# sksundaram-learning/linkerd

Hardware: AMD Instinct MI355X
Metric: histogram samples ingested+summarized/sec (1M series) and % HBM peak (higher is better)
Workload: dtype u32; 1 GPU; C3: 1M series, 1e9 Zipf(s=1) samples per step, log-normal values; series_total=1000000, series_per_gpu=1000000, rotating_batches=3, parallelism=series-sharded x1 (weighted ranges), step=ingest (sample+plan+bin1+bin2) + snapshot(reset, dense counts + summaries)

## Files before the change

### linkerd_amd/csrc/l5dh_ingest.hip

```cpp
#include <algorithm>
#include <type_traits>

#include "l5dh_device.hpp"

namespace l5dh {
namespace {

constexpr uint32_t RSAMPLE = 1u << 18;
#ifndef L5DH_RS_WG
#define L5DH_RS_WG 64
#endif
constexpr int RS_WG = L5DH_RS_WG;
static_assert((RSAMPLE + RS_WG - 1) / RS_WG <= 65535, "k_rsample's u16 LDS counters: at most 65535 draws per workgroup");
constexpr uint32_t INVALID = 0xFFFFFFFFu;

__device__ __forceinline__ uint32_t round_up(uint32_t x, uint32_t m) { return (x + m - 1) / m * m; }

__device__ __forceinline__ uint32_t rcap(double prev, double e, double s, bool exact, double pad, uint32_t align,
                                         uint32_t pct, double z, bool floor_sample) {
  double c;
  if (exact) {
    c = e;
  } else {
    const double e0 = prev / s, sg = sqrt(e0 + 1.0);
    const double r = sqrt(e + 1.0) + 0.5 * z;
    const double sb = !floor_sample && prev == 0.0 && e == 0.0 ? ceil(4.0 * s) : ceil(r * r * s);
    if (prev > 0.0 && e >= e0 - 6.0 * sg && (floor_sample || e <= e0 + 4.0 * sg)) {
      c = ceil(prev * 1.0625 + 4.0 * sqrt(prev));
      if (floor_sample) c = fmax(c, sb);
    } else {
      c = sb;
    }
    c += pad;
  }
  if (pct != 100) c = floor(c * (double)pct / 100.0);
  return round_up((uint32_t)fmin(c, 1073741824.0), align);
}

__device__ __forceinline__ uint64_t block_excl_scan64(uint64_t v, uint64_t* lds , uint64_t* total) {
  const int lane = threadIdx.x & 63, w = threadIdx.x >> 6;
  const uint64_t incl = wave_incl_scan(v);
  if (lane == 63) lds[w] = incl;
  __syncthreads();
  if (threadIdx.x == 0) {
    uint64_t acc = 0;
    for (int k = 0; k < 16; ++k) {
      const uint64_t q = lds[k];
      lds[k] = acc;
      acc += q;
    }
    lds[16] = acc;
  }
  __syncthreads();
  const uint64_t r = lds[w] + incl - v;
  *total = lds[16];
  __syncthreads();
  return r;
}

#ifdef L5DH_PHASES
__device__ unsigned long long g_phase_plan[16];
#define RP_MARK(k) \
  if (threadIdx.x == 0) g_phase_plan[k] = wall_clock64();
#define RS_MARK(k) \
  if (threadIdx.x == 0 && blockIdx.x == 0) g_phase_plan[k] = wall_clock64();
#else
#define RP_MARK(k)
#define RS_MARK(k)
#endif

__global__ __launch_bounds__(1024) void k_rsample(const uint32_t* __restrict__ series, size_t n, uint32_t S, uint32_t K,
                                                  uint32_t* __restrict__ kest) {
  extern __shared__ uint32_t c[];
  RS_MARK(8)
  for (uint32_t i = threadIdx.x; i < (K + 1) / 2; i += 1024) c[i] = 0;
  __syncthreads();
  RS_MARK(9)
  const uint64_t m = n < RSAMPLE ? n : RSAMPLE;
  const uint64_t per = (m + RS_WG - 1) / RS_WG;
  const uint64_t k0 = blockIdx.x * per, k1 = k0 + per < m ? k0 + per : m;
  for (uint64_t kb = k0; kb < k1; kb += 4 * 1024) {
    uint32_t sv[4];
#pragma unroll
    for (int u = 0; u < 4; ++u) {
      const uint64_t k = kb + threadIdx.x + 1024u * u;
      const uint64_t i = m == n ? k : k * n / m;
      sv[u] = k < k1 ? series[i < n ? i : 0] : 0xFFFFFFFFu;
    }
#pragma unroll
    for (int u = 0; u < 4; ++u)
      if (sv[u] < S) {
        const uint32_t key = sv[u] >> 4;
        atomicAdd(&c[key >> 1], (key & 1u) ? 0x10000u : 1u);
      }
  }
  __syncthreads();
  RS_MARK(10)
  for (uint32_t i = threadIdx.x; i < (K + 1) / 2; i += 1024) {
    const uint32_t x = c[i];
    if (x & 0xFFFFu) atomicAdd(&kest[2 * i], x & 0xFFFFu);
    if ((x >> 16) && 2 * i + 1 < K) atomicAdd(&kest[2 * i + 1], x >> 16);
  }
  RS_MARK(11)
}

constexpr size_t RPLAN1_LDS = 32768 * 4;
constexpr uint32_t RFIX2_ONE_WG_MAX = 16384;
__global__ __launch_bounds__(1024) void k_rplan1(size_t n, uint32_t F, const uint32_t* __restrict__ kest,
                                                 const uint32_t* __restrict__ kprev, uint32_t* __restrict__ meta,
                                                 size_t cap32, size_t dlim16, uint32_t thr_min, uint32_t dmax,
                                                 uint32_t pct) {
  __shared__ uint32_t lh[33];
  __shared__ uint32_t sthr;
  __shared__ uint4 lds4[17];
  __shared__ uint64_t l64[17];
  __shared__ uint32_t dl[DIRECT_MAX + 1];
  __shared__ uint32_t capl[BIN1_BINS];
  extern __shared__ uint32_t tw[];
  const MetaLayout L = meta_layout(F);
  const uint32_t FS = (F + ST_TILES - 1) / ST_TILES;
  const uint32_t NW = (F + 31) / 32;
  const uint64_t m = n < RSAMPLE ? n : RSAMPLE;
  const bool exact = m == n;
  const double s = m ? (double)n / (double)m : 1.0;
  const uint32_t j = threadIdx.x, t0 = j * 32;
  const int lane = lane_id();
  RP_MARK(0)
  if (j < 33) lh[j] = 0;
  capl[j] = 0;
  auto load_pairs = [&](const uint32_t* __restrict__ kw, uint4 (&x)[16]) {
#pragma unroll
    for (int i = 0; i < 16; ++i) {
      const uint32_t t = 2u * (j + 1024u * (uint32_t)i);
      x[i] = make_uint4(0u, 0u, 0u, 0u);
      if (t + 1 < F) {
        x[i] = *reinterpret_cast<const uint4*>(kw + 2 * t);
      } else if (t < F) {
        x[i].x = kw[2 * t];
        x[i].y = kw[2 * t + 1];
      }
    }
  };
  uint2 te[16];
  {
    uint4 x[16];
    load_pairs(kest, x);
#pragma unroll
    for (int i = 0; i < 16; ++i) te[i] = make_uint2(x[i].x + x[i].y, x[i].z + x[i].w);
  }
  auto scaled = [&](uint32_t v) -> uint32_t { return (uint32_t)fmin((double)v * s, 4294967295.0); };
  __syncthreads();
  RP_MARK(1)
  auto hist = [&](uint32_t v) {
    const uint32_t e = scaled(v);
    const bool ok = dmax > 0 && e >= thr_min && e > 0;
    const int bin = ok ? 31 - __clz((int)e) : 0;
    const uint64_t act = __ballot(ok);
    if (!act) return;
    const int b0 = __builtin_amdgcn_readlane(bin, __builtin_ctzll(act));
    if (__ballot(ok && bin == b0) == act) {
      if (lane == 0) atomicAdd(&lh[b0], (uint32_t)__popcll(act));
    } else if (ok) {
      atomicAdd(&lh[bin], 1u);
    }
  };
#pragma unroll
  for (int i = 0; i < 16; ++i) {
    hist(te[i].x);
    hist(te[i].y);
  }
  __syncthreads();
  if (j < 64) {
    const uint32_t c = j < 32 ? lh[31 - j] : 0u;
    const uint32_t cum = wave_incl_scan32(c);
    const uint64_t ok = __ballot(dmax > 0 && j < 32 && cum <= dmax);
    const int nb = __popcll(ok);
    if (j == 0) sthr = nb ? max(max(thr_min, 1u), 1u << (32 - nb)) : 0xFFFFFFFFu;
  }
#pragma unroll
  for (int i = 0; i < 16; ++i) reinterpret_cast<uint2*>(tw)[j + 1024u * (uint32_t)i] = te[i];
  uint4 xp[16];
  load_pairs(kprev, xp);
  __syncthreads();
  const uint32_t thr = sthr;
  RP_MARK(2)
  uint32_t dbits = 0, E = 0;
#pragma unroll
  for (int k = 0; k < 32; ++k) {
    const uint32_t kk = (uint32_t)(k + (int)j) & 31u;
    const uint32_t v = tw[t0 + kk];
    if (t0 + kk < F && scaled(v) >= thr) dbits |= 1u << kk;
    else E += v;
  }
  __syncthreads();
#pragma unroll
  for (int i = 0; i < 16; ++i)
    reinterpret_cast<uint2*>(tw)[j + 1024u * (uint32_t)i] = make_uint2(xp[i].x + xp[i].y, xp[i].z + xp[i].w);
  __syncthreads();
  uint64_t P = 0;
#pragma unroll
  for (int k = 0; k < 32; ++k) {
    const uint32_t kk = (uint32_t)(k + (int)j) & 31u;
    if (!((dbits >> kk) & 1u)) P += tw[t0 + kk];
  }
  RP_MARK(3)
  uint32_t cv[4] = {(uint32_t)__popc(dbits), 0u, 0u, 0u}, ct[4];
  block_excl_scan4<1024>(cv, lds4, ct);
  const uint32_t ND = ct[0];
  meta[L.dbits() + j] = j < NW ? dbits : 0u;
  meta[L.dpre() + j] = cv[0];
  {
    uint32_t x = dbits, di = cv[0];
    while (x) {
      const uint32_t k = (uint32_t)(__ffs((int)x) - 1);
      x &= x - 1u;
      dl[di] = t0 + k;
      meta[L.dlist() + di] = t0 + k;
      ++di;
    }
  }
  P += __shfl_xor(P, 1, 64);
  E += __shfl_xor(E, 1, 64);
  RP_MARK(4)
  if ((j & 1u) == 0 && (j >> 1) < FS) {
    const uint32_t b = j >> 1;
    capl[b] = rcap((double)P, (double)E, s, exact, 256.0, 4, pct, 6.0, true);
    meta[L.btot() + b] = (uint32_t)min(P, (uint64_t)0xFFFFFFFFu);
  }
  __syncthreads();
  RP_MARK(5)
  const uint32_t TB = FS + 2 * ND;
  if (j >= FS && j < TB) {
    const uint32_t t = dl[(j - FS) >> 1], h = (j - FS) & 1u;
    const double p = (double)kprev[2 * t + h], e = (double)kest[2 * t + h];
    capl[j] = rcap(p, e, s, exact, 256.0, 8, pct, 5.0, false);
  }
  __syncthreads();
  const bool stb = j < FS, dj = j >= FS && j < TB;
  uint64_t tot32, tot16;
  const uint64_t base32 = block_excl_scan64(stb ? (uint64_t)capl[j] : 0ull, l64, &tot32);
  const uint64_t base16 = block_excl_scan64(dj ? (uint64_t)capl[j] : 0ull, l64, &tot16);
  const uint64_t base = stb ? base32 : base16;
  const uint64_t lim = stb ? cap32 : dlim16;
  if (base + capl[j] + 16 > lim)
    capl[j] = base + 16 < lim ? (uint32_t)(lim - 16 - base) & (stb ? ~3u : ~7u) : 0u;
  meta[L.bbase() + j] = (uint32_t)base;
  meta[L.bcap() + j] = j < TB ? capl[j] : 0u;
  meta[L.bcnt() + j] = 0u;
  if (j == 0) {
    uint32_t* hdr = meta + L.hdr();
    hdr[H_ND] = ND;
    hdr[H_OV1] = 0;
    hdr[H_REDO1] = 0;
    hdr[H_OV2] = 0;
    hdr[H_REDO2] = 0;
    hdr[H_COUNT2] = 0;
    hdr[H_EXACT] = exact ? 1u : 0u;
    hdr[H_D16] = (uint32_t)min(tot16, (uint64_t)dlim16);
  }
  RP_MARK(6)
}

#ifdef L5DH_PHASES
__device__ unsigned long long g_phase1[1024 * 8];
__device__ unsigned long long g_phase3[1024 * 8];
#define PH_INIT                                                            \
  const bool ph_on = threadIdx.x == 0 || threadIdx.x == NT1 - 64;          \
  uint32_t ph_acc[8] = {0, 0, 0, 0, 0, 0, 0, 0}, ph_t = (uint32_t)wall_clock64();
#define PH_VWAIT asm volatile("s_waitcnt vmcnt(0)" ::: "memory");
#define PH_MARK(k)                                 \
  if (ph_on) {                                     \
    const uint32_t ph_n = (uint32_t)wall_clock64(); \
    ph_acc[k] += ph_n - ph_t;                      \
    ph_t = ph_n;                                   \
  }
#define PH_FLUSH                                                                          \
  if (ph_on && pass == 0 && (threadIdx.x == 0 || gridDim.x <= 256)) {                      \
    const uint32_t ph_row = blockIdx.x + (threadIdx.x ? 512u : 0u);                       \
    for (int k = 0; k < 7; ++k) g_phase1[ph_row * 8 + k] += ph_acc[k];                    \
    g_phase1[ph_row * 8 + 7] += 1;                                                        \
    if (gridDim.x <= 256) {                                                               \
      g_phase1[(768 + blockIdx.x) * 8 + (threadIdx.x ? 1 : 0)] += ph_acc[7];              \
      if (threadIdx.x == 0) g_phase1[(768 + blockIdx.x) * 8 + 7] += 1;                    \
    }                                                                                     \
  }
#else
#define PH_INIT
#define PH_MARK(k)
#define PH_VWAIT
#define PH_FLUSH
#endif
__device__ __forceinline__ uint4 ld_stream(const uint32_t* p) { return *reinterpret_cast<const uint4*>(p); }
constexpr int CHW = 16384;
constexpr int NT1 = 1024;
constexpr int B1_PT = CHW / NT1;
constexpr int B1_PH = B1_PT / 2;
constexpr int B1_GS = 4;
constexpr int B1_HG = B1_PH / 4;
static_assert(B1_PH % 4 == 0 && B1_PH % B1_GS == 0 && B1_GS % 4 == 0, "halves of whole 16-B groups");
static_assert(NT1 == BIN1_BINS, "one bin per thread");
constexpr uint32_t DSUM_PMAX = 1u << 17;
static_assert(DSUM_PMAX == 1u << 17, "the ranking loop tests the bits of 2^17f, 0x48000000");
constexpr uint32_t NODEST = 0xFFFFFFFFu - (uint32_t)CHW;
constexpr int DSUM_N = DIRECT_MAX * TILE;

struct Bin1Lds {
  static constexpr int DW_N = 1024;
  static constexpr size_t o_stage = 0;
  static constexpr size_t o_cnt = o_stage + CHW * 4;
  static constexpr size_t o_offr = o_cnt + BIN1_BINS * 4;
  static constexpr size_t o_rdelta = o_offr + BIN1_BINS * 4;
  static constexpr size_t o_heads = o_rdelta + BIN1_BINS * 4;
  static constexpr size_t o_gpre = o_heads + CHW / 32 * 4;
  static constexpr size_t o_dw = o_gpre + CHW / 64 * 2;
  static constexpr size_t o_lut2 = o_dw + DW_N * 8;
  static constexpr size_t o_dsum = o_lut2 + LUT2_N * 8;
  static constexpr size_t o_dacc = o_dsum + DSUM_N * 4;
  static constexpr size_t o_breg = o_dacc + BIN1_BINS * 4;
  static constexpr size_t bytes = o_breg + BIN1_BINS * 8;

  template <typename T>
  static __device__ __forceinline__ T* at(uint32_t* smem, size_t o) {
    return reinterpret_cast<T*>(reinterpret_cast<char*>(smem) + o);
  }
  static __device__ __forceinline__ uint32_t* stage(uint32_t* smem) { return at<uint32_t>(smem, o_stage); }
  static __device__ __forceinline__ uint32_t* cnt(uint32_t* smem) { return at<uint32_t>(smem, o_cnt); }
  static __device__ __forceinline__ uint32_t* offr(uint32_t* smem) { return at<uint32_t>(smem, o_offr); }
  static __device__ __forceinline__ uint32_t* rdelta(uint32_t* smem) { return at<uint32_t>(smem, o_rdelta); }
  static __device__ __forceinline__ uint32_t* heads(uint32_t* smem) { return at<uint32_t>(smem, o_heads); }
  static __device__ __forceinline__ uint16_t* gpre(uint32_t* smem) { return at<uint16_t>(smem, o_gpre); }
  static __device__ __forceinline__ uint2* dw(uint32_t* smem) { return at<uint2>(smem, o_dw); }
  static __device__ __forceinline__ uint2* lut2(uint32_t* smem) { return at<uint2>(smem, o_lut2); }
  static __device__ __forceinline__ uint32_t* dsum(uint32_t* smem) { return at<uint32_t>(smem, o_dsum); }
  static __device__ __forceinline__ uint32_t* dacc(uint32_t* smem) { return at<uint32_t>(smem, o_dacc); }
  static __device__ __forceinline__ uint2* breg(uint32_t* smem) { return at<uint2>(smem, o_breg); }
};
static_assert(Bin1Lds::bytes <= 160 * 1024, "one workgroup's LDS");
static_assert(Bin1Lds::o_stage % 16 == 0 && Bin1Lds::o_heads % 16 == 0 && Bin1Lds::o_dw % 16 == 0 &&
                  Bin1Lds::o_lut2 % 16 == 0 && Bin1Lds::o_breg % 16 == 0,
              "stage and heads are accessed as uint4, dw, lut2 and breg as uint2");
static_assert(2ull * CHW * (DSUM_PMAX - 1) < (1ull << 32),
              "u32 direct sums: <= CHW (2^17 - 1) at a sub-chunk's start + as much from the sub-chunk");

static_assert(CHW <= 32768 && BIN1_BINS <= 1024, "15-bit ranks, 10-bit bins");
__device__ __forceinline__ uint32_t pk_make(uint32_t rank, uint32_t bin) { return rank | (bin << 15); }
__device__ __forceinline__ uint32_t pk_rank(uint32_t pk) { return pk & 0x7FFFu; }
__device__ __forceinline__ uint32_t pk_bin(uint32_t pk) { return (pk >> 15) & 1023u; }
static_assert(CHW < 65536, "16-bit stage offsets");
__device__ __forceinline__ uint32_t offr_make(uint32_t off, uint32_t run) { return off | (run << 16); }
__device__ __forceinline__ uint32_t offr_off(uint32_t w) { return w & 0xFFFFu; }
__device__ __forceinline__ uint32_t offr_run(uint32_t w) { return w >> 16; }

struct Bin1Run {
  uint32_t n, old;
  uint32_t base, cap;
};

__device__ __forceinline__ uint32_t b1_slot(uint32_t c0, int kk, int q) {
  return c0 + 4u * ((uint32_t)kk * NT1 + threadIdx.x) + (uint32_t)q;
}

struct Bin1Regs {
  uint4 s[B1_HG], v[B1_HG];
};
struct Bin1Half {
  uint32_t s[B1_PH];
  float f[B1_PH];
};

__device__ __forceinline__ Bin1Regs b1_issue_half(const uint32_t* series, const float* values, uint32_t c0, int h) {
  Bin1Regs r;
#pragma unroll
  for (int k = 0; k < B1_HG; ++k) {
    const uint32_t base = b1_slot(c0, h * B1_HG + k, 0);
    r.s[k] = ld_stream(series + base);
    r.v[k] = ld_stream(reinterpret_cast<const uint32_t*>(values) + base);
  }
  return r;
}

__device__ __forceinline__ Bin1Half b1_unpack_half(Bin1Regs r) {
  Bin1Half x;
#pragma unroll
  for (int k = 0; k < B1_HG; ++k) {
    const uint4 s4 = r.s[k], u4 = r.v[k];
    const float4 f4 = make_float4(__uint_as_float(u4.x), __uint_as_float(u4.y), __uint_as_float(u4.z),
                                  __uint_as_float(u4.w));
    x.s[4 * k] = s4.x; x.s[4 * k + 1] = s4.y; x.s[4 * k + 2] = s4.z; x.s[4 * k + 3] = s4.w;
    x.f[4 * k] = f4.x; x.f[4 * k + 1] = f4.y; x.f[4 * k + 2] = f4.z; x.f[4 * k + 3] = f4.w;
  }
  return x;
}
__device__ __forceinline__ Bin1Half b1_load_ragged(const uint32_t* series, const float* values, uint32_t c0,
                                                   uint32_t hi, int h) {
  Bin1Half x;
#pragma unroll
  for (int k = 0; k < B1_PH; ++k) {
    const uint32_t i = b1_slot(c0, h * B1_HG + (k >> 2), k & 3);
    const bool in = i < hi;
    x.s[k] = in ? series[i] : 0xFFFFFFFFu;
    x.f[k] = in ? values[i] : 0.0f;
  }
  return x;
}
__device__ __forceinline__ bool b1_ragged_invalid(Bin1Half x, uint32_t c0, uint32_t hi, int h, uint32_t S) {
  bool bad = false;
#pragma unroll
  for (int k = 0; k < B1_PH; ++k) bad |= b1_slot(c0, h * B1_HG + (k >> 2), k & 3) < hi && x.s[k] >= S;
  return bad;
}
__device__ __forceinline__ bool b1_group_invalid(Bin1Half x, int g, uint32_t S) {
  bool bad = false;
#pragma unroll
  for (int q = 0; q < B1_GS; ++q) bad |= x.s[g + q] >= S;
  return bad;
}

static_assert(B1_PT / B1_GS == 4, "one priority level per group of a sub-chunk");
__device__ __forceinline__ void b1_progress_prio(int gi) {
  if (gi == 0) __builtin_amdgcn_s_setprio(3);
  else if (gi == 1) __builtin_amdgcn_s_setprio(2);
  else if (gi == 2) __builtin_amdgcn_s_setprio(1);
  else __builtin_amdgcn_s_setprio(0);
}

static_assert(B1_GS == 4, "a group's pk words are returned as a uint4");
__device__ __forceinline__ uint4 b1_rank_group(uint32_t* smem, int h, int g, Bin1Half x, const uint32_t* series,
                                               const float* values, uint32_t c0, uint32_t S, uint32_t FS, uint32_t TB,
                                               Tables tb, int64_t* sumfix, int pass) {
  uint32_t* const stage = Bin1Lds::stage(smem);
  uint32_t* const cnt = Bin1Lds::cnt(smem);
  uint2* const dw = Bin1Lds::dw(smem);
  uint2* const lut2 = Bin1Lds::lut2(smem);
  uint32_t* const dsum = Bin1Lds::dsum(smem);
  constexpr int GS = B1_GS;
  uint32_t pl[GS], pk[GS];
  uint32_t escm = 0;
#pragma unroll
  for (int q = 0; q < GS; ++q) {
    const float f = x.f[g + q];
    const bool fast = __float_as_uint(f) < 0x48000000u;
    pl[q] = fast ? (uint32_t)f : 0u;
    escm |= (!fast && x.s[g + q] < S) ? (1u << q) : 0u;
  }
  if (__ballot(escm != 0u)) {
#pragma unroll 1
    for (int q = 0; q < GS; ++q) {
      if ((escm >> q) & 1u) {
        const uint32_t i = b1_slot(c0, h * B1_HG + (g + q) / 4, q & 3);
        const uint32_t si = series[i];
        const uint32_t r = payload1_slow(si, values[i], tb, pass == 0 ? sumfix : nullptr);
        if (pass == 0 && r - DSUM_PMAX < V_ESC - DSUM_PMAX) {
          const uint2 d = dw[(si >> (TILE_SHIFT + 5)) & 1023u];
          if ((d.x >> ((si >> TILE_SHIFT) & 31u)) & 1u)
            atomicAdd(reinterpret_cast<unsigned long long*>(&sumfix[si]), (unsigned long long)r);
        }
#pragma unroll
        for (int u = 0; u < GS; ++u) pl[u] = q == u ? r : pl[u];
      }
    }
  }
  uint2 dv[GS], lv[GS];
#pragma unroll
  for (int q = 0; q < GS; ++q) dv[q] = dw[(x.s[g + q] >> (TILE_SHIFT + 5)) & 1023u];
#pragma unroll
  for (int q = 0; q < GS; ++q) lv[q] = lut2[lut2_index(pl[q])];
  uint32_t rc4[GS];
#pragma unroll
  for (int q = 0; q < GS; ++q) {
    const uint32_t s = x.s[g + q];
    const uint32_t tw = __builtin_amdgcn_ubfe(s, TILE_SHIFT, 5);
    const bool direct = s < S && __builtin_amdgcn_ubfe(dv[q].x, tw, 1) != 0u;
    const uint32_t di = dv[q].y + (uint32_t)__popc(__builtin_amdgcn_ubfe(dv[q].x, 0, tw));
    const uint32_t p = pl[q];
    uint32_t o;
    const uint32_t bk = lut2_decode(p, lv[q], o);
    const bool esc = p >= V_ESC;
    const uint32_t bucket = sel_u32(esc, p - V_ESC, bk);
    rc4[q] = sel_u32(direct, ((s & (TILE - 1)) << 11) | bucket, ((s & (ST_TILES * TILE - 1)) << 21) | p);
    const uint32_t dbin = FS + 2u * di + ((s >> 4) & 1u);
    const uint32_t bn = sel_u32(s < S, sel_u32(direct, dbin, s >> ST_SHIFT), TB);
    pk[q] = pk_make(atomicAdd(cnt + bn, 1u), bn);
    if (direct && pass == 0 && p - 1u < DSUM_PMAX - 1u) atomicAdd(&dsum[di * TILE + (s & (TILE - 1))], p);
  }
#pragma unroll
  for (int j = 0; j < GS / 4; ++j)
    *reinterpret_cast<uint4*>(stage + b1_slot(0u, h * B1_HG + g / 4 + j, 0)) =
        make_uint4(rc4[4 * j], rc4[4 * j + 1], rc4[4 * j + 2], rc4[4 * j + 3]);
  asm volatile("" ::: "memory");
  return make_uint4(pk[0], pk[1], pk[2], pk[3]);
}

__device__ __forceinline__ Bin1Run b1_reserve_run(uint32_t* smem, uint32_t tq, uint32_t TB, uint32_t* bcnt) {
  uint32_t* const cnt = Bin1Lds::cnt(smem);
  uint2* const breg = Bin1Lds::breg(smem);
  Bin1Run r;
  r.n = tq <= TB ? cnt[tq] : 0u;
  r.old = 0;
  const uint2 reg = breg[tq];
  r.base = reg.x;
  r.cap = reg.y;
  if (tq < TB && r.n) r.old = atomicAdd(&bcnt[tq], r.n);
  return r;
}

__device__ __forceinline__ void b1_guard_flush(uint32_t* smem, uint32_t tq, uint32_t rn, uint32_t FS, uint32_t TB,
                                               const uint32_t* meta, uint32_t dlist, uint32_t S, int64_t* sumfix) {
  uint32_t* const dsum = Bin1Lds::dsum(smem);
  uint32_t* const dacc = Bin1Lds::dacc(smem);
  bool fl = false;
  if (tq >= FS && tq < TB && rn) {
    const uint32_t A = dacc[tq] + rn;
    fl = A > (uint32_t)CHW;
    dacc[tq] = fl ? 0u : A;
  }
  for (uint64_t fm = __ballot(fl); fm; fm &= fm - 1) {
    const uint32_t fb = (tq & ~63u) + (uint32_t)__builtin_ctzll(fm) - FS;
    if ((tq & 63u) < TILE / 2) {
      const uint32_t h = fb * (TILE / 2) + (tq & 63u);
      const uint32_t v = dsum[h];
      dsum[h] = 0;
      const uint32_t sr = meta[dlist + h / TILE] * TILE + (h & (TILE - 1));
      if (v && sr < S) atomicAdd(reinterpret_cast<unsigned long long*>(&sumfix[sr]), (unsigned long long)v);
    }
  }
}

__device__ __forceinline__ uint32_t b1_scan_waves(uint32_t pv, uint32_t tq, uint32_t* wsum) {
  const uint32_t wi = wave_incl_scan32(pv);
  if ((tq & 63u) == 63u) wsum[tq >> 6] = wi;
  return wi;
}
__device__ __forceinline__ void b1_scan_heads(uint32_t* smem, const uint32_t* wsum, int wv, uint32_t pv, uint32_t wi,
                                              uint32_t rn) {
  uint32_t* const offr = Bin1Lds::offr(smem);
  uint32_t* const heads = Bin1Lds::heads(smem);
  uint32_t pre = 0;
  for (int q = 0; q < wv; ++q) pre += wsum[q];
  const uint32_t ex = pre + wi - pv;
  offr[threadIdx.x] = ex;
  if (rn) atomicOr(&heads[offr_off(ex) >> 5], 1u << (ex & 31u));
}

__device__ __forceinline__ void b1_read_slots(uint32_t* smem, uint32_t (&rec)[B1_PT]) {
  uint32_t* const stage = Bin1Lds::stage(smem);
#pragma unroll
  for (int kk = 0; kk < B1_PT / 4; ++kk) {
    const uint4 v = *reinterpret_cast<const uint4*>(stage + b1_slot(0u, kk, 0));
    rec[4 * kk] = v.x; rec[4 * kk + 1] = v.y; rec[4 * kk + 2] = v.z; rec[4 * kk + 3] = v.w;
  }
}

__device__ __forceinline__ void b1_scatter(uint32_t* smem, uint32_t pk, uint32_t rec) {
  uint32_t* const stage = Bin1Lds::stage(smem);
  uint32_t* const offr = Bin1Lds::offr(smem);
  stage[offr_off(offr[pk_bin(pk)]) + pk_rank(pk)] = rec;
}

__device__ __forceinline__ void b1_group_prefixes(uint32_t* smem, int lane) {
  uint32_t* const heads = Bin1Lds::heads(smem);
  uint16_t* const gpre = Bin1Lds::gpre(smem);
  constexpr int GPL = CHW / 64 / 64;
  static_assert(GPL % 2 == 0, "two groups per 16-B read");
  uint32_t pc[GPL], t = 0;
#pragma unroll
  for (int k = 0; k < GPL; k += 2) {
    const uint4 w = *reinterpret_cast<const uint4*>(heads + 2u * (GPL * (uint32_t)lane + (uint32_t)k));
    pc[k] = (uint32_t)(__popc(w.x) + __popc(w.y));
    pc[k + 1] = (uint32_t)(__popc(w.z) + __popc(w.w));
    t += pc[k] + pc[k + 1];
  }
  uint32_t ex = wave_incl_scan32(t) - t;
#pragma unroll
  for (int k = 0; k < GPL; ++k) {
    gpre[GPL * (uint32_t)lane + (uint32_t)k] = (uint16_t)ex;
    ex += pc[k];
  }
}

__device__ __forceinline__ void b1_run_delta(uint32_t* smem, const Bin1Run& r, uint32_t TB, uint32_t* hdr) {
  uint32_t* const offr = Bin1Lds::offr(smem);
  uint32_t* const rdelta = Bin1Lds::rdelta(smem);
  const uint32_t b = threadIdx.x;
  if (r.n) {
    uint32_t d = NODEST;
    if (b < TB) {
      if (r.old + r.n <= r.cap) d = r.base + r.old - offr_off(offr[b]);
      else hdr[H_OV1] = 1u;
    }
    rdelta[offr_run(offr[b])] = d;
  }
}

__device__ __forceinline__ void b1_write_out(uint32_t* smem, int wv, int lane, uint32_t nst, uint32_t* rec32,
                                             uint16_t* rec16) {
  uint32_t* const stage = Bin1Lds::stage(smem);
  uint32_t* const rdelta = Bin1Lds::rdelta(smem);
  uint32_t* const heads = Bin1Lds::heads(smem);
  uint16_t* const gpre = Bin1Lds::gpre(smem);
#pragma unroll 4
  for (int k = 0; k < B1_PT; ++k) {
    const uint32_t i = (uint32_t)wv * (B1_PT * 64) + (uint32_t)k * 64 + (uint32_t)lane;
    const uint32_t g = i >> 6;
    const unsigned long long hw = *reinterpret_cast<const unsigned long long*>(heads + 2 * g);
    const uint32_t run = (uint32_t)gpre[g] + mask_below(hw) + (uint32_t)((hw >> lane) & 1ull) - 1u;
    const uint32_t d = rdelta[run];
    if (d != NODEST) {
      if (run < nst)
        rec32[i + d] = stage[i];
      else
        rec16[i + d] = (uint16_t)stage[i];
    }
  }
}

__device__ __forceinline__ void b1_flush_sums(uint32_t* smem, uint32_t ND, const uint32_t* dlist, uint32_t S,
                                              int64_t* sumfix) {
  uint32_t* const dsum = Bin1Lds::dsum(smem);
  for (uint32_t i = threadIdx.x; i < ND * TILE; i += NT1) {
    const unsigned long long v = dsum[i];
    const uint32_t s = dlist[i / TILE] * TILE + (i & (TILE - 1));
    if (v && s < S) atomicAdd(reinterpret_cast<unsigned long long*>(&sumfix[s]), (unsigned long long)v);
  }
}

__global__ __launch_bounds__(NT1) void k_rbin1w(const uint32_t* __restrict__ series, const float* __restrict__ values,
                                                size_t n, size_t per, uint32_t S, uint32_t F, Tables tb,
                                                uint32_t* __restrict__ meta, uint32_t* __restrict__ rec32,
                                                uint16_t* __restrict__ rec16, int64_t* __restrict__ sumfix,
                                                uint32_t* __restrict__ err, int vec, int pass) {
  extern __shared__ __attribute__((aligned(16))) uint32_t smem[];
  __shared__ uint32_t wsum[NT1 / 64];
  uint32_t* const cnt = Bin1Lds::cnt(smem);
  uint32_t* const offr = Bin1Lds::offr(smem);
  uint32_t* const heads = Bin1Lds::heads(smem);
  uint2* const dw = Bin1Lds::dw(smem);
  uint2* const lut2 = Bin1Lds::lut2(smem);
  uint32_t* const dsum = Bin1Lds::dsum(smem);
  uint32_t* const dacc = Bin1Lds::dacc(smem);
  uint2* const breg = Bin1Lds::breg(smem);
  const MetaLayout L = meta_layout(F);
  uint32_t* hdr = meta + L.hdr();
  if (pass == 1 && __builtin_amdgcn_readfirstlane(hdr[H_REDO1]) == 0u) return;
  uint32_t* bcnt = meta + L.bcnt();
  const uint32_t* bbase = meta + L.bbase();
  const uint32_t* bcap = meta + L.bcap();
  const uint32_t* dlist = meta + L.dlist();
  const uint32_t FS = (F + ST_TILES - 1) / ST_TILES;
  const uint32_t NW = (F + 31) / 32;
  const uint32_t ND = hdr[H_ND];
  const uint32_t TB = FS + 2 * ND;
  const int lane = lane_id();
  const int wv = threadIdx.x >> 6;
  for (uint32_t w = threadIdx.x; w < NW; w += NT1) dw[w] = make_uint2(meta[L.dbits() + w], meta[L.dpre() + w]);
  cnt[threadIdx.x] = 0;
  dacc[threadIdx.x] = 0;
  for (uint32_t i = threadIdx.x; i < LUT2_N; i += NT1) lut2[i] = tb.lut2[i];
  for (uint32_t i = threadIdx.x; i < ND * TILE; i += NT1) dsum[i] = 0;
  __syncthreads();
  const uint32_t lo = (uint32_t)((size_t)blockIdx.x * per);
  const uint32_t hi = (uint32_t)min((size_t)lo + per, n);
  bool bad = false;
  {
    const uint32_t b = threadIdx.x;
    breg[b] = b < TB ? make_uint2(bbase[b], bcap[b]) : make_uint2(0u, 0u);
  }
  PH_INIT
  Bin1Regs pf;
  if (vec && lo + (uint32_t)CHW <= hi) pf = b1_issue_half(series, values, lo, 0);
  for (uint32_t c0 = lo; c0 < hi; c0 += CHW) {
    for (uint32_t wd = threadIdx.x; wd < CHW / 32; wd += NT1) heads[wd] = 0u;
    uint32_t pk[B1_PT];
    const bool full = vec && c0 + (uint32_t)CHW <= hi;
    Bin1Regs sh;
#pragma unroll
    for (int h = 0; h < 2; ++h) {
      if (h == 1) { PH_MARK(1) }
      Bin1Half hf;
      if (full) {
        hf = b1_unpack_half(h == 0 ? pf : sh);
      } else {
        hf = b1_load_ragged(series, values, c0, hi, h);
        bad |= b1_ragged_invalid(hf, c0, hi, h, S);
      }
      if (full) {
        PH_VWAIT
        if (h == 0) { PH_MARK(0) } else { PH_MARK(2) }
      }
#pragma unroll
      for (int g = 0; g < B1_PH; g += B1_GS) {
        if (h == 0 && g == B1_GS && full) sh = b1_issue_half(series, values, c0, 1);
        b1_progress_prio(h * (B1_PH / B1_GS) + g / B1_GS);
        if (full) bad |= b1_group_invalid(hf, g, S);
        const uint4 p4 = b1_rank_group(smem, h, g, hf, series, values, c0, S, FS, TB, tb, sumfix, pass);
        pk[h * B1_PH + g] = p4.x; pk[h * B1_PH + g + 1] = p4.y; pk[h * B1_PH + g + 2] = p4.z; pk[h * B1_PH + g + 3] = p4.w;
      }
    }
    PH_MARK(3)
    __syncthreads();
    PH_MARK(7)
    uint32_t tq = threadIdx.x;
    asm volatile("" : "+v"(tq));
    const Bin1Run run = b1_reserve_run(smem, tq, TB, bcnt);
    if (pass == 0) b1_guard_flush(smem, tq, run.n, FS, TB, meta, L.dlist(), S, sumfix);
    const uint32_t pv = offr_make(run.n, run.n ? 1u : 0u);
    const uint32_t wi = b1_scan_waves(pv, tq, wsum);
    __syncthreads();
    b1_scan_heads(smem, wsum, wv, pv, wi, run.n);
    uint32_t rec[B1_PT];
    b1_read_slots(smem, rec);
    __syncthreads();
    PH_MARK(4)
    if (vec && c0 + 2u * (uint32_t)CHW <= hi) pf = b1_issue_half(series, values, c0 + (uint32_t)CHW, 0);
#pragma unroll
    for (int k = 0; k < B1_PT; ++k) b1_scatter(smem, pk[k], rec[k]);
    if (wv == 0) b1_group_prefixes(smem, lane);
    b1_run_delta(smem, run, TB, hdr);
    __syncthreads();
    PH_MARK(5)
    const uint32_t nst = offr_run(offr[FS]);
    cnt[threadIdx.x] = 0;
    b1_write_out(smem, wv, lane, nst, rec32, rec16);
    __syncthreads();
    PH_MARK(6)
  }
  PH_FLUSH
  if (pass == 0) {
    b1_flush_sums(smem, ND, dlist, S, sumfix);
    if (bad) atomicAdd(err, 1u);
  }
}

__device__ __forceinline__ uint32_t lut3_byte(uint32_t v) {
  const uint32_t sh = 25u - (uint32_t)__builtin_clz(v | 64u);
  return ((v >> sh) + (sh << 6)) << 3;
}
__device__ __forceinline__ uint32_t lut3_bucket(uint32_t v, uint2 x) {
  return (x.x & 0x7FFu) + (((v << 11) | 0x7FFu) >= x.x ? 1u : 0u) + (v >= x.y ? 1u : 0u);
}

__global__ __launch_bounds__(1024) void k_rfix1(uint32_t F, uint32_t* __restrict__ meta, const uint32_t* __restrict__ err,
                                                uint32_t* __restrict__ err_host) {
  __shared__ uint32_t lds[17];
  const MetaLayout L = meta_layout(F);
  uint32_t* hdr = meta + L.hdr();
  if (threadIdx.x == 0) *reinterpret_cast<volatile uint32_t*>(err_host) = *err;
  const uint32_t FS = (F + ST_TILES - 1) / ST_TILES;
  const uint32_t ND = hdr[H_ND];
  const uint32_t TB = FS + 2 * ND;
  const uint32_t ov = hdr[H_OV1];
  const uint32_t b = threadIdx.x;
  const bool stb = b < FS, dj = b >= FS && b < TB;
  const uint32_t c = b < TB ? meta[L.bcnt() + b] : 0u;
  if (stb && !hdr[H_EXACT]) {
    const double P = (double)meta[L.btot() + b];
    if ((double)c > P * 1.0625 + 4.0 * sqrt(P) + 256.0) hdr[H_COUNT2] = 1u;
  }
  meta[L.btot() + b] = c;
  uint32_t t32, t16;
  const uint32_t nb32 = block_excl_scan<1024>(stb ? round_up(c, 4) : 0u, lds, &t32);
  const uint32_t nb16 = block_excl_scan<1024>(dj ? round_up(c, 8) : 0u, lds, &t16);
  const uint32_t nb = stb ? nb32 : nb16;
  const uint32_t base = ov ? nb : meta[L.bbase() + b];
  if (dj) {
    const uint32_t t = meta[L.dlist() + ((b - FS) >> 1)], h = (b - FS) & 1u;
    meta[L.kbase() + 2 * t + h] = base;
    meta[L.kcnt() + 2 * t + h] = c;
  }
  if (ov) {
    meta[L.bbase() + b] = nb;
    meta[L.bcap() + b] = round_up(c, stb ? 4 : 8);
    meta[L.bcnt() + b] = 0u;
  }
  const uint32_t d16 = hdr[H_D16];
  if (ov && t16 > d16) {
    for (uint32_t k = b; k < L.K; k += 1024)
      if (!((meta[L.dbits() + (k >> 6)] >> ((k >> 1) & 31u)) & 1u)) meta[L.kcap() + k] = 0u;
  }
  uint32_t all;
  const uint32_t is = block_excl_scan<1024>(stb ? (c + ITEM2 - 1) / ITEM2 : 0u, lds, &all);
  if (stb) meta[L.istart() + b] = is;
  __syncthreads();
  if (b == 0) {
    meta[L.istart() + FS] = all;
    hdr[H_ITEMS] = all;
    if (ov && t16 > d16) {
      hdr[H_D16] = t16;
      hdr[H_COUNT2] = 1u;
    }
    hdr[H_OV2] = 0u;
    hdr[H_REDO2] = 0u;
    hdr[H_REDO1] = ov;
    hdr[H_OV1] = 0u;
    if (ov) hdr[H_NOVR1] += 1u;
  }
}

__device__ __forceinline__ bool tile_direct(const uint32_t* __restrict__ meta, const MetaLayout& L, uint32_t t) {
  return (meta[L.dbits() + (t >> 5)] >> (t & 31u)) & 1u;
}

__device__ __forceinline__ uint64_t wsum_before(const uint64_t* __restrict__ ws, uint32_t b, uint64_t* red ) {
  uint64_t v = threadIdx.x < b ? ws[threadIdx.x] : 0ull;
  v = wave_sum(v);
  if ((threadIdx.x & 63) == 0) red[threadIdx.x >> 6] = v;
  __syncthreads();
  uint64_t r = 0;
  for (int q = 0; q < 16; ++q) r += red[q];
  __syncthreads();
  return r;
}

__global__ __launch_bounds__(1024) void k_rplan2a(size_t n, uint32_t F, uint32_t* __restrict__ kest,
                                                  const uint32_t* __restrict__ kprev, uint32_t* __restrict__ meta,
                                                  uint32_t pct) {
  __shared__ uint64_t red[16];
  const MetaLayout L = meta_layout(F);
  const uint64_t m = n < RSAMPLE ? n : RSAMPLE;
  const bool exact = m == n;
  const double s = m ? (double)n / (double)m : 1.0;
  const uint32_t k = blockIdx.x * 1024u + threadIdx.x;
  uint32_t cap = 0;
  if (k < L.K) {
    const uint32_t e = kest[k];
    if (e) kest[k] = 0;
    if (!tile_direct(meta, L, k >> 1)) {
      cap = rcap((double)kprev[k], (double)e, s, exact, 32.0, 8, pct, 5.0, false);
      meta[L.kcap() + k] = cap;
    }
  }
  const uint64_t w = wave_sum((uint64_t)cap);
  if ((threadIdx.x & 63) == 0) red[threadIdx.x >> 6] = w;
  __syncthreads();
  if (threadIdx.x == 0) {
    uint64_t t = 0;
    for (int q = 0; q < 16; ++q) t += red[q];
    reinterpret_cast<uint64_t*>(meta + L.wsum())[blockIdx.x] = t;
  }
}

__global__ __launch_bounds__(1024) void k_rplan2b(uint32_t F, uint32_t* __restrict__ meta, size_t cap16) {
  __shared__ uint64_t red[16];
  __shared__ uint64_t l64[17];
  const MetaLayout L = meta_layout(F);
  uint32_t* hdr = meta + L.hdr();
  const uint64_t before = wsum_before(reinterpret_cast<const uint64_t*>(meta + L.wsum()), blockIdx.x, red);
  const uint32_t k = blockIdx.x * 1024u + threadIdx.x;
  const bool mine = k < L.K && !tile_direct(meta, L, k >> 1);
  uint32_t cap = mine ? meta[L.kcap() + k] : 0u;
  uint64_t total;
  const uint64_t base = hdr[H_D16] + before + block_excl_scan64((uint64_t)cap, l64, &total);
  if (mine) {
    if (base + cap + 64 > cap16) {
      cap = base + 64 < cap16 ? (uint32_t)(cap16 - 64 - base) & ~7u : 0u;
      hdr[H_COUNT2] = 1u;
    }
    meta[L.kbase() + k] = (uint32_t)base;
    meta[L.kcap() + k] = cap;
    meta[L.kcnt() + k] = 0u;
  }
}

constexpr int B2_KEYS = 2 * ST_TILES;
constexpr int B2_NT = 512, B2_PER_CU = 2;
constexpr size_t rbin2_lds() {
  return 2048 * 8 + LUT2_N * 8 + 2 * B2_KEYS * 8 + (B2_KEYS + 64) * 4 + 2 * (size_t)ITEM2 * 4;
}

template <int NT>
__global__ __launch_bounds__(NT, B2_PER_CU * NT / 256) void k_rbin2(uint32_t S, uint32_t F, Tables tb, uint32_t* __restrict__ meta,
                                                 const uint32_t* __restrict__ m_is, const uint32_t* __restrict__ m_bb,
                                                 const uint32_t* __restrict__ m_bt,
                                                 const uint32_t* __restrict__ rec32, uint16_t* __restrict__ rec16,
                                                 int64_t* __restrict__ sumfix, int pass) {
  constexpr int PT = (int)ITEM2 / NT;
  constexpr int PG = PT / 4;
  __shared__ __attribute__((aligned(16))) uint32_t smem[rbin2_lds() / 4];
  unsigned long long* lsum = reinterpret_cast<unsigned long long*>(smem);
  uint2* lut3 = reinterpret_cast<uint2*>(lsum + 2048);
  uint2* ocx = lut3 + LUT2_N;
  uint32_t* cnt = reinterpret_cast<uint32_t*>(ocx + 2 * B2_KEYS);
  uint32_t* stage = cnt + B2_KEYS + 64;
  const MetaLayout L = meta_layout(F);
  uint32_t* hdr = meta + L.hdr();
  if (pass == 1 && __builtin_amdgcn_readfirstlane(hdr[H_REDO2]) == 0u) return;
  const uint32_t nitems = hdr[H_ITEMS];
  const uint32_t i0 = (uint32_t)(((uint64_t)blockIdx.x * nitems) / gridDim.x);
  const uint32_t i1 = (uint32_t)(((uint64_t)(blockIdx.x + 1) * nitems) / gridDim.x);
  if (i0 >= i1) return;
  const uint32_t FS = (F + ST_TILES - 1) / ST_TILES;
  uint32_t* kcnt = meta + L.kcnt();
  const uint32_t* kbase = meta + L.kbase();
  const uint32_t* kcap = meta + L.kcap();
  const int lane = lane_id(), wv = threadIdx.x >> 6;
  for (int i = threadIdx.x; i < LUT2_N; i += NT) lut3[i] = tb.lut3[i];
  for (int i = threadIdx.x; i < 2048; i += NT) lsum[i] = 0ull;
  for (int i = threadIdx.x; i < B2_KEYS; i += NT) cnt[i] = 0u;
  uint32_t jl = 0, jh = FS;
  while (jh - jl > 1) {
    const uint32_t mid = (jl + jh) >> 1;
    if (m_is[mid] <= i0) jl = mid; else jh = mid;
  }
  __syncthreads();
  uint32_t jn = jl;
  auto item_range = [&](uint32_t item, uint32_t& j, uint32_t& a, uint32_t& e) {
    while (m_is[jn + 1] <= item) jn = __builtin_amdgcn_readfirstlane(jn + 1);
    j = jn;
    const uint32_t bb = m_bb[jn];
    a = bb + (item - m_is[jn]) * ITEM2;
    e = min(a + ITEM2, bb + m_bt[jn]);
  };
  auto load = [&](uint32_t a, uint32_t e, uint4 (&x)[PG]) {
#pragma unroll
    for (int g = 0; g < PG; ++g) {
      const uint32_t idx = a + 4u * ((uint32_t)g * NT + threadIdx.x);
      x[g] = *reinterpret_cast<const uint4*>(rec32 + (idx < e ? idx : a));
    }
  };
  uint32_t cur_j = 0xFFFFFFFFu;
  auto flush = [&](uint32_t jj) {
    for (int i = threadIdx.x; i < 2048; i += NT) {
      const unsigned long long v = lsum[i];
      const uint32_t s = jj * 2048u + (uint32_t)i;
      if (v && s < S) atomicAdd(reinterpret_cast<unsigned long long*>(&sumfix[s]), v);
      lsum[i] = 0ull;
    }
  };
  if (pass == 0 && __builtin_amdgcn_readfirstlane(hdr[H_COUNT2]) != 0u) {
    uint32_t j, a, e;
    item_range(i0, j, a, e);
    uint4 x[PG];
    load(a, e, x);
    for (uint32_t item = i0; item < i1; ++item) {
      const uint32_t cj = j, ctot = e - a;
      uint4 xn[PG];
      if (item + 1 < i1) item_range(item + 1, j, a, e);
      load(a, e, xn);
      if (cj != cur_j) {
        if (cur_j != 0xFFFFFFFFu) {
          __syncthreads();
          flush(cur_j);
        }
        cur_j = cj;
        __syncthreads();
      }
#pragma unroll
      for (int g = 0; g < PG; ++g) {
        const uint32_t rr[4] = {x[g].x, x[g].y, x[g].z, x[g].w};
#pragma unroll
        for (int q = 0; q < 4; ++q) {
          const uint32_t p = rr[q] & 0x1FFFFFu;
          const bool valid = 4u * ((uint32_t)g * NT + threadIdx.x) + (uint32_t)q < ctot;
          atomicAdd(&cnt[valid ? rr[q] >> 25 : (uint32_t)B2_KEYS + (uint32_t)lane], 1u);
          atomicAdd(&lsum[(rr[q] >> 21) & 2047u], (unsigned long long)((valid && p < V_ESC) ? p : 0u));
        }
      }
      __syncthreads();
      if (wv < 2) {
        const uint32_t rk = (uint32_t)wv * 64u + (uint32_t)lane;
        const uint32_t rc = cnt[rk];
        if (rc) atomicAdd(&kcnt[cj * (uint32_t)B2_KEYS + rk], rc);
        cnt[rk] = 0u;
      }
      __syncthreads();
#pragma unroll
      for (int g = 0; g < PG; ++g) x[g] = xn[g];
    }
    __syncthreads();
    flush(cur_j);
    return;
  }
  auto write_out = [&](int bb, uint32_t total) {
    const uint32_t* st = stage + bb * ITEM2;
    const uint2* oc = ocx + bb * B2_KEYS;
    constexpr int WB = 4;
#pragma unroll
    for (int k0 = 0; k0 < PT; k0 += WB) {
      uint32_t x[WB];
      uint2 o[WB];
#pragma unroll
      for (int j = 0; j < WB; ++j) x[j] = st[(uint32_t)wv * (PT * 64) + (uint32_t)(k0 + j) * 64 + (uint32_t)lane];
#pragma unroll
      for (int j = 0; j < WB; ++j) o[j] = oc[(x[j] >> 16) & (B2_KEYS - 1)];
#pragma unroll
      for (int j = 0; j < WB; ++j) {
        const uint32_t i = (uint32_t)wv * (PT * 64) + (uint32_t)(k0 + j) * 64 + (uint32_t)lane;
        if (i < total && o[j].y != INVALID) rec16[o[j].y + (i - o[j].x)] = (uint16_t)(x[j] & 0xFFFFu);
      }
      __builtin_amdgcn_sched_barrier(0);
    }
  };
  uint32_t j, a, e;
  item_range(i0, j, a, e);
  uint4 x[PG];
  load(a, e, x);
  uint32_t prev_total = 0;
#ifdef L5DH_PHASES
  unsigned long long ph2[5] = {0, 0, 0, 0, 0}, ph2_t = wall_clock64();
#define PH2_MARK(k)                                  \
  if (threadIdx.x == 0) {                            \
    const unsigned long long ph_n = wall_clock64();  \
    ph2[k] += ph_n - ph2_t;                          \
    ph2_t = ph_n;                                    \
  }
#else
#define PH2_MARK(k)
#endif
  for (uint32_t item = i0; item < i1; ++item) {
    const int b = (int)(item & 1u);
    const uint32_t cj = j, ctot = e - a;
    uint4 xn[PG];
    if (item + 1 < i1) item_range(item + 1, j, a, e);
    load(a, e, xn);
    if (cj != cur_j) {
      if (pass == 0 && cur_j != 0xFFFFFFFFu) {
        __syncthreads();
        flush(cur_j);
      }
      cur_j = cj;
      __syncthreads();
    }
    uint32_t kr[PT], rank[PT];
    {
      uint32_t r[PT];
#pragma unroll
      for (int g = 0; g < PG; ++g) {
        r[4 * g] = x[g].x; r[4 * g + 1] = x[g].y; r[4 * g + 2] = x[g].z; r[4 * g + 3] = x[g].w;
      }
      bool escq = false;
#pragma unroll
      for (int k = 0; k < PT; ++k) escq |= (r[k] & 0x1FFFFFu) >= V_ESC;
      const bool lean = ctot == ITEM2 && pass == 0 && !__ballot(escq);
      constexpr int H = PT / 2;
      if (lean) {
#pragma unroll
        for (int k = 0; k < PT; ++k) {
          uint2 lv[H];
          if (k % H == 0) {
#pragma unroll
            for (int q = 0; q < H; ++q) lv[q] = lut3[lut3_byte(r[k + q] & 0x1FFFFFu) >> 3];
          }
          const uint32_t p = r[k] & 0x1FFFFFu;
          kr[k] = ((r[k] >> 25) << 16) | ((r[k] >> 10) & 0xF800u) | lut3_bucket(p, lv[k % H]);
          rank[k] = atomicAdd(&cnt[r[k] >> 25], 1u);
          atomicAdd(&lsum[(r[k] >> 21) & 2047u], (unsigned long long)p);
        }
      } else {
#pragma unroll
        for (int k = 0; k < PT; ++k) {
          uint2 lv[H];
          if (k % H == 0) {
#pragma unroll
            for (int q = 0; q < H; ++q) lv[q] = lut3[lut3_byte(r[k + q] & 0x1FFFFFu) >> 3];
          }
          const uint32_t p = r[k] & 0x1FFFFFu;
          const bool esc = p >= V_ESC;
          const uint32_t bucket = sel_u32(esc, p - V_ESC, lut3_bucket(p, lv[k % H]));
          const bool valid = 4u * ((uint32_t)(k >> 2) * NT + threadIdx.x) + (uint32_t)(k & 3) < ctot;
          kr[k] = valid ? (((r[k] >> 25) << 16) | ((r[k] >> 10) & 0xF800u) | bucket) : NOKEY;
          rank[k] = atomicAdd(&cnt[valid ? r[k] >> 25 : (uint32_t)B2_KEYS + (uint32_t)lane], 1u);
          atomicAdd(&lsum[(r[k] >> 21) & 2047u], (unsigned long long)((pass == 0 && valid && !esc) ? p : 0u));
        }
      }
    }
    __syncthreads();
    PH2_MARK(0)
    uint32_t rc = 0, rold = 0, rbase = 0, rcapv = 0;
    const uint32_t rk = (uint32_t)wv * 64u + (uint32_t)lane;
    if (wv < 2) {
      const uint32_t gk = cj * (uint32_t)B2_KEYS + rk;
      rc = cnt[rk];
      if (rc) {
        rold = atomicAdd(&kcnt[gk], rc);
        rbase = kbase[gk];
        rcapv = kcap[gk];
      }
    } else if (wv == 2) {
      const uint32_t c0 = cnt[2 * lane], c1 = cnt[2 * lane + 1];
      const uint32_t ex = wave_incl_scan32(c0 + c1) - (c0 + c1);
      ocx[b * B2_KEYS + 2 * lane].x = ex;
      ocx[b * B2_KEYS + 2 * lane + 1].x = ex + c0;
    }
    __syncthreads();
    PH2_MARK(1)
    {
      uint32_t* st = stage + b * ITEM2;
      const uint2* oc = ocx + b * B2_KEYS;
#pragma unroll
      for (int k0 = 0; k0 < PT; k0 += 4) {
        uint32_t o[4];
#pragma unroll
        for (int j = 0; j < 4; ++j) o[j] = oc[(kr[k0 + j] >> 16) & (B2_KEYS - 1)].x;
#pragma unroll
        for (int j = 0; j < 4; ++j)
          *(kr[k0 + j] != NOKEY ? &st[o[j] + rank[k0 + j]] : &cnt[B2_KEYS + lane]) = kr[k0 + j];
      }
    }
    PH2_MARK(2)
    if (item > i0) write_out(b ^ 1, prev_total);
    PH2_MARK(3)
    if (wv < 2) {
      uint32_t rb = INVALID;
      if (rc) {
        if (rold + rc <= rcapv) rb = rbase + rold;
        else hdr[H_OV2] = 1u;
      }
      ocx[b * B2_KEYS + rk].y = rb;
      cnt[rk] = 0u;
    }
    __syncthreads();
    PH2_MARK(4)
    prev_total = ctot;
#pragma unroll
    for (int g = 0; g < PG; ++g) x[g] = xn[g];
  }
  write_out((int)((i1 - 1) & 1u), prev_total);
  __syncthreads();
  if (pass == 0) flush(cur_j);
#ifdef L5DH_PHASES
  if (threadIdx.x == 0 && pass == 0) {
    for (int k = 0; k < 5; ++k) g_phase3[blockIdx.x * 8 + k] += ph2[k];
    g_phase3[blockIdx.x * 8 + 7] += 1;
  }
#endif
}

__global__ __launch_bounds__(1024) void k_rfix2a(uint32_t F, uint32_t* __restrict__ meta, uint32_t* __restrict__ kprev) {
  __shared__ uint64_t red[16];
  const MetaLayout L = meta_layout(F);
  uint32_t* hdr = meta + L.hdr();
  const uint32_t k = blockIdx.x * 1024u + threadIdx.x;
  uint32_t r8 = 0;
  if (k < L.K) {
    const uint32_t c = meta[L.kcnt() + k];
    kprev[k] = c;
    if (!tile_direct(meta, L, k >> 1)) r8 = round_up(c, 8);
  }
  const uint64_t w = wave_sum((uint64_t)r8);
  if ((threadIdx.x & 63) == 0) red[threadIdx.x >> 6] = w;
  __syncthreads();
  if (threadIdx.x == 0) {
    uint64_t t = 0;
    for (int q = 0; q < 16; ++q) t += red[q];
    reinterpret_cast<uint64_t*>(meta + L.wsum())[blockIdx.x] = t;
    if (blockIdx.x == 0) hdr[H_REDO2] = hdr[H_OV2] | hdr[H_COUNT2];
  }
}

__global__ __launch_bounds__(1024) void k_rfix2b(uint32_t F, uint32_t* __restrict__ meta) {
  __shared__ uint64_t red[16];
  __shared__ uint64_t l64[17];
  const MetaLayout L = meta_layout(F);
  uint32_t* hdr = meta + L.hdr();
  if (hdr[H_REDO2] == 0u) return;
  const uint64_t before = wsum_before(reinterpret_cast<const uint64_t*>(meta + L.wsum()), blockIdx.x, red);
  const uint32_t k = blockIdx.x * 1024u + threadIdx.x;
  const bool mine = k < L.K && !tile_direct(meta, L, k >> 1);
  const uint32_t c8 = mine ? round_up(meta[L.kcnt() + k], 8) : 0u;
  uint64_t total;
  const uint64_t base = hdr[H_D16] + before + block_excl_scan64((uint64_t)c8, l64, &total);
  if (mine) {
    meta[L.kbase() + k] = (uint32_t)base;
    meta[L.kcap() + k] = c8;
    meta[L.kcnt() + k] = 0u;
  }
  if (blockIdx.x == 0 && threadIdx.x == 0) {
    if (hdr[H_COUNT2]) hdr[H_NCNT2] += 1u;
    else hdr[H_NOVR2] += 1u;
    hdr[H_OV2] = 0u;
  }
}

__global__ __launch_bounds__(1024) void k_rfix2s(uint32_t F, uint32_t* __restrict__ meta, uint32_t* __restrict__ kprev) {
  __shared__ uint64_t l64[17];
  const MetaLayout L = meta_layout(F);
  uint32_t* hdr = meta + L.hdr();
  constexpr uint32_t KPM = RFIX2_ONE_WG_MAX / 1024;
  const uint32_t KP = (L.K + 1023) / 1024, k0 = threadIdx.x * KP;
  const uint32_t redo = hdr[H_OV2] | hdr[H_COUNT2];
  const uint32_t counted = hdr[H_COUNT2];
  uint32_t c8[KPM], dm = 0;
  uint64_t mine = 0;
#pragma unroll
  for (uint32_t q = 0; q < KPM; ++q) {
    const uint32_t k = k0 + q;
    c8[q] = 0;
    if (q < KP && k < L.K) {
      const uint32_t c = meta[L.kcnt() + k];
      kprev[k] = c;
      if (tile_direct(meta, L, k >> 1)) {
        dm |= 1u << q;
      } else {
        c8[q] = round_up(c, 8);
        mine += c8[q];
      }
    }
  }
  __syncthreads();
  if (threadIdx.x == 0) hdr[H_REDO2] = redo;
  if (!redo) return;
  uint64_t total;
  uint64_t kb = (uint64_t)hdr[H_D16] + block_excl_scan64(mine, l64, &total);
#pragma unroll
  for (uint32_t q = 0; q < KPM; ++q) {
    const uint32_t k = k0 + q;
    if (q < KP && k < L.K && !((dm >> q) & 1u)) {
      meta[L.kbase() + k] = (uint32_t)kb;
      meta[L.kcap() + k] = c8[q];
      meta[L.kcnt() + k] = 0u;
      kb += c8[q];
    }
  }
  if (threadIdx.x == 0) {
    if (counted) hdr[H_NCNT2] += 1u;
    else hdr[H_NOVR2] += 1u;
    hdr[H_OV2] = 0u;
  }
}

__global__ __launch_bounds__(256) void k_fetch_host(const uint32_t* __restrict__ hs, const uint32_t* __restrict__ hv,
                                                    uint32_t* __restrict__ ds, uint32_t* __restrict__ dv, size_t n) {
  const size_t stride = (size_t)gridDim.x * blockDim.x;
  for (size_t i = (size_t)blockIdx.x * blockDim.x + threadIdx.x; i < n; i += stride) {
    const uint32_t s = hs[i], v = hv[i];
    ds[i] = s;
    dv[i] = v;
  }
}

}

#ifdef L5DH_PHASES
extern "C" __attribute__((visibility("default"))) int l5dh_dev_phases3(unsigned long long* out) {
  return (int)hipMemcpyFromSymbol(out, HIP_SYMBOL(g_phase3), sizeof(g_phase3), 0, hipMemcpyDeviceToHost);
}
extern "C" __attribute__((visibility("default"))) int l5dh_dev_phases_plan(unsigned long long* out) {
  return (int)hipMemcpyFromSymbol(out, HIP_SYMBOL(g_phase_plan), sizeof(g_phase_plan), 0, hipMemcpyDeviceToHost);
}
extern "C" __attribute__((visibility("default"))) int l5dh_dev_phases1(unsigned long long* out) {
  return (int)hipMemcpyFromSymbol(out, HIP_SYMBOL(g_phase1), sizeof(g_phase1), 0, hipMemcpyDeviceToHost);
}
#endif

hipError_t launch_fetch_host(const uint32_t* hs, const uint32_t* hv, uint32_t* ds, uint32_t* dv, size_t n,
                             hipStream_t st) {
  if (n == 0) return hipSuccess;
  const size_t blocks = std::min<size_t>((n + 255) / 256, 2048);
  hipLaunchKernelGGL(k_fetch_host, dim3((unsigned)blocks), dim3(256), 0, st, hs, hv, ds, dv, n);
  return hipGetLastError();
}

hipError_t set_ingest_attributes() {
  hipError_t e;
  if ((e = hipFuncSetAttribute((const void*)k_rsample, hipFuncAttributeMaxDynamicSharedMemorySize, 32768 * 4)))
    return e;
  if ((e = hipFuncSetAttribute((const void*)k_rplan1, hipFuncAttributeMaxDynamicSharedMemorySize, (int)RPLAN1_LDS)))
    return e;
  return hipFuncSetAttribute((const void*)k_rbin1w, hipFuncAttributeMaxDynamicSharedMemorySize, (int)Bin1Lds::bytes);
}

hipError_t launch_ingest(const IngestArgs& a, int stage, hipStream_t st) {
  const uint32_t K = 2 * a.F;
  switch (stage) {
    case 0:
      hipLaunchKernelGGL(k_rsample, dim3(RS_WG), dim3(1024), (size_t)((K + 1) / 2) * 4, st, a.series, a.n, a.S, K,
                         a.kest);
      hipLaunchKernelGGL(k_rplan1, dim3(1), dim3(1024), RPLAN1_LDS, st, a.n, a.F, a.kest, a.kprev, a.meta, a.cap32,
                         a.dlim16, a.thr_min, a.dmax, a.pct);
      {
        const uint32_t B = (K + 1023) / 1024;
        hipLaunchKernelGGL(k_rplan2a, dim3(B), dim3(1024), 0, st, a.n, a.F, a.kest, a.kprev, a.meta, a.pct);
        hipLaunchKernelGGL(k_rplan2b, dim3(B), dim3(1024), 0, st, a.F, a.meta, a.cap16);
      }
      break;
    case 1:
      for (int pass = 0; pass < 2; ++pass) {
        hipLaunchKernelGGL(k_rbin1w, dim3(a.G), dim3(NT1), Bin1Lds::bytes, st, a.series, a.values, a.n, a.per, a.S, a.F,
                           a.tb, a.meta, a.rec32, a.rec16, a.sumfix, a.err, a.vec ? 1 : 0, pass);
        if (pass == 0) hipLaunchKernelGGL(k_rfix1, dim3(1), dim3(1024), 0, st, a.F, a.meta, a.err, a.err_host);
      }
      break;
    case 2:
      break;
    default: {
      const uint32_t B = (K + 1023) / 1024;
      for (int pass = 0; pass < 2; ++pass) {
        const MetaLayout L = meta_layout(a.F);
        hipLaunchKernelGGL(k_rbin2<B2_NT>, dim3(a.num_cu * B2_PER_CU), dim3(B2_NT), 0, st, a.S, a.F, a.tb, a.meta,
                           a.meta + L.istart(), a.meta + L.bbase(), a.meta + L.btot(), a.rec32, a.rec16, a.sumfix,
                           pass);
        if (pass == 0 && K <= RFIX2_ONE_WG_MAX) {
          hipLaunchKernelGGL(k_rfix2s, dim3(1), dim3(1024), 0, st, a.F, a.meta, a.kprev);
        } else if (pass == 0) {
          hipLaunchKernelGGL(k_rfix2a, dim3(B), dim3(1024), 0, st, a.F, a.meta, a.kprev);
          hipLaunchKernelGGL(k_rfix2b, dim3(B), dim3(1024), 0, st, a.F, a.meta);
        }
      }
      break;
    }
  }
  return hipGetLastError();
}

}
```

Before: 182.6 billion samples/s.

## Issue next-chunk prefetch earlier in bin1 and make loads unconditional

Moves the prefetch of the next chunk's first half from after the scan barriers into the last rank group of the current chunk, so the global loads overlap more of the ranking, scatter and write-out work. Loads become unconditional, with invalid chunks pointing at a spare buffer, which removes branches around the prefetch. Empty asm 'arrive' fences pin where the loaded registers are consumed so the compiler cannot sink or hoist the waits. The cost is higher register pressure from keeping the prefetched half live across barriers and the scatter phase, plus extra dummy loads on ragged or final chunks.

```diff
diff --git a/linkerd_amd/csrc/l5dh_ingest.hip b/linkerd_amd/csrc/l5dh_ingest.hip
--- a/linkerd_amd/csrc/l5dh_ingest.hip
+++ b/linkerd_amd/csrc/l5dh_ingest.hip
@@ -368,15 +368,29 @@
   float f[B1_PH];
 };
 
-__device__ __forceinline__ Bin1Regs b1_issue_half(const uint32_t* series, const float* values, uint32_t c0, int h) {
+__device__ __forceinline__ Bin1Regs b1_issue_half(const uint32_t* series, const float* values, uint32_t c0, int h,
+                                                  bool ok, const uint32_t* spare) {
   Bin1Regs r;
 #pragma unroll
   for (int k = 0; k < B1_HG; ++k) {
     const uint32_t base = b1_slot(c0, h * B1_HG + k, 0);
-    r.s[k] = ld_stream(series + base);
-    r.v[k] = ld_stream(reinterpret_cast<const uint32_t*>(values) + base);
+    r.s[k] = ld_stream(ok ? series + base : spare);
+    r.v[k] = ld_stream(ok ? reinterpret_cast<const uint32_t*>(values) + base : spare);
   }
   return r;
+}
+static_assert(B1_HG == 2 && B1_PH == 8, "the arrive points name a half's 16 registers");
+__device__ __forceinline__ void b1_arrive(Bin1Regs& r) {
+  asm volatile(""
+               : "+v"(r.s[0].x), "+v"(r.s[0].y), "+v"(r.s[0].z), "+v"(r.s[0].w), "+v"(r.s[1].x), "+v"(r.s[1].y),
+                 "+v"(r.s[1].z), "+v"(r.s[1].w), "+v"(r.v[0].x), "+v"(r.v[0].y), "+v"(r.v[0].z), "+v"(r.v[0].w),
+                 "+v"(r.v[1].x), "+v"(r.v[1].y), "+v"(r.v[1].z), "+v"(r.v[1].w));
+}
+__device__ __forceinline__ void b1_arrive(Bin1Half& x) {
+  asm volatile(""
+               : "+v"(x.s[0]), "+v"(x.s[1]), "+v"(x.s[2]), "+v"(x.s[3]), "+v"(x.s[4]), "+v"(x.s[5]), "+v"(x.s[6]),
+                 "+v"(x.s[7]), "+v"(x.f[0]), "+v"(x.f[1]), "+v"(x.f[2]), "+v"(x.f[3]), "+v"(x.f[4]), "+v"(x.f[5]),
+                 "+v"(x.f[6]), "+v"(x.f[7]));
 }
 
 __device__ __forceinline__ Bin1Half b1_unpack_half(Bin1Regs r) {
@@ -448,8 +462,10 @@
     for (int q = 0; q < GS; ++q) {
       if ((escm >> q) & 1u) {
         const uint32_t i = b1_slot(c0, h * B1_HG + (g + q) / 4, q & 3);
-        const uint32_t si = series[i];
-        const uint32_t r = payload1_slow(si, values[i], tb, pass == 0 ? sumfix : nullptr);
+        uint32_t si = series[i];
+        float vi = values[i];
+        asm volatile("" : "+v"(si), "+v"(vi));
+        const uint32_t r = payload1_slow(si, vi, tb, pass == 0 ? sumfix : nullptr);
         if (pass == 0 && r - DSUM_PMAX < V_ESC - DSUM_PMAX) {
           const uint2 d = dw[(si >> (TILE_SHIFT + 5)) & 1023u];
           if ((d.x >> ((si >> TILE_SHIFT) & 31u)) & 1u)
@@ -666,8 +682,9 @@
     breg[b] = b < TB ? make_uint2(bbase[b], bcap[b]) : make_uint2(0u, 0u);
   }
   PH_INIT
-  Bin1Regs pf;
-  if (vec && lo + (uint32_t)CHW <= hi) pf = b1_issue_half(series, values, lo, 0);
+  const uint32_t* const spare = reinterpret_cast<const uint32_t*>(tb.lim_pad);
+  Bin1Regs pf = b1_issue_half(series, values, lo, 0, vec && lo + (uint32_t)CHW <= hi, spare);
+  b1_arrive(pf);
   for (uint32_t c0 = lo; c0 < hi; c0 += CHW) {
     for (uint32_t wd = threadIdx.x; wd < CHW / 32; wd += NT1) heads[wd] = 0u;
     uint32_t pk[B1_PT];
@@ -681,6 +698,7 @@
         hf = b1_unpack_half(h == 0 ? pf : sh);
       } else {
         hf = b1_load_ragged(series, values, c0, hi, h);
+        b1_arrive(hf);
         bad |= b1_ragged_invalid(hf, c0, hi, h, S);
       }
       if (full) {
@@ -689,7 +707,9 @@
       }
 #pragma unroll
       for (int g = 0; g < B1_PH; g += B1_GS) {
-        if (h == 0 && g == B1_GS && full) sh = b1_issue_half(series, values, c0, 1);
+        if (h == 0 && g == B1_GS) sh = b1_issue_half(series, values, c0, 1, full, spare);
+        if (h == 1 && g == B1_PH - B1_GS)
+          pf = b1_issue_half(series, values, c0 + (uint32_t)CHW, 0, vec && c0 + 2u * (uint32_t)CHW <= hi, spare);
         b1_progress_prio(h * (B1_PH / B1_GS) + g / B1_GS);
         if (full) bad |= b1_group_invalid(hf, g, S);
         const uint4 p4 = b1_rank_group(smem, h, g, hf, series, values, c0, S, FS, TB, tb, sumfix, pass);
@@ -711,7 +731,6 @@
     b1_read_slots(smem, rec);
     __syncthreads();
     PH_MARK(4)
-    if (vec && c0 + 2u * (uint32_t)CHW <= hi) pf = b1_issue_half(series, values, c0 + (uint32_t)CHW, 0);
 #pragma unroll
     for (int k = 0; k < B1_PT; ++k) b1_scatter(smem, pk[k], rec[k]);
     if (wv == 0) b1_group_prefixes(smem, lane);
@@ -720,6 +739,7 @@
     PH_MARK(5)
     const uint32_t nst = offr_run(offr[FS]);
     cnt[threadIdx.x] = 0;
+    b1_arrive(pf);
     b1_write_out(smem, wv, lane, nst, rec32, rec16);
     __syncthreads();
     PH_MARK(6)
```

Measured after the change: 185.3 billion samples/s, median of 6. 1.01x the previous value.
